# flavie-yuan-liu/DL_attack_on_ImageNet

Hardware: AMD Instinct MI355X
Metric: adversarial images/sec (ADiL learning step, classifier included) (higher is better)
Workload: dtype bf16; 1 GPU; ADiL learn_dictionary_a step vs resnet50, 512 images/GPU, 50 atoms, 224x224, bf16 image streams + fp32 D/V master, loss=logits, clean pseudo-labels computed once per image and cached (1 fwd + 1 bwd per step; result-neutral, profiles/r03_label_stability.md); global_batch=512, atoms=50, inner_iters=132, parallelism=dp1: images+codes sharded, D replicated, 1 all-reduce(grad_d)/step

## Files before the change

dl_attack_on_imagenet_amd/csrc/adil_stem.hip:

```cpp
#include <hip/hip_runtime.h>
#include <stdint.h>

#include "adil_common.h"
#include "adil_hip.h"
#include "adil_mfma.h"

namespace {

struct StemNorm { float mean[3]; float inv_std[3]; };

#define ST_T 16
#define ST_ROWS (2 * ST_T + 5)
#define ST_COLS 40
#define ST_RS (ST_COLS * 4 + 8)
#define ST_K 224
#define ST_WS (ST_K + 8)
#define ST_OS 72

template <typename TX>
__global__ __launch_bounds__(256) __attribute__((amdgpu_waves_per_eu(3))) void stem_conv_fwd_kernel(const TX* __restrict__ x, const bf16_t* __restrict__ wf,
                                                            StemNorm nm, const float* __restrict__ scale,
                                                            const float* __restrict__ shift, bf16_t* __restrict__ y,
                                                            int H, int W, int OH, int OW) {
    __shared__ __attribute__((aligned(16))) bf16_t smem[ST_ROWS * ST_RS + 64 * ST_WS];
    static_assert(4 * 32 * ST_OS <= ST_ROWS * ST_RS + 64 * ST_WS, "output scratch must fit in the tile buffers");
    bf16_t* sin = smem;
    bf16_t* sw = smem + ST_ROWS * ST_RS;
    bf16_t* sout = smem;
    const int tid = threadIdx.x, lane = tid & 63, w = tid >> 6, c = lane & 31, h = lane >> 5;
    const int n = blockIdx.z, oh0 = blockIdx.y * ST_T, ow0 = blockIdx.x * ST_T;
    {
        u32x4 wv[7];
#pragma unroll
        for (int j = 0; j < 7; ++j) wv[j] = *reinterpret_cast<const u32x4*>(wf + (size_t)(tid + 256 * j) * 8);
#pragma unroll
        for (int j = 0; j < 7; ++j) {
            const int q = tid + 256 * j, co = q / 28, off = q - co * 28;
            *reinterpret_cast<u32x4*>(sw + co * ST_WS + off * 8) = wv[j];
        }
    }
    const TX* xn = x + (size_t)n * 3 * H * W;
    constexpr int NPOS = (ST_ROWS * ST_COLS + 255) / 256;
    float raw[NPOS][3], okm[NPOS];
#pragma unroll
    for (int j = 0; j < NPOS; ++j) {
        const int pos = tid + 256 * j < ST_ROWS * ST_COLS ? tid + 256 * j : ST_ROWS * ST_COLS - 1;
        const int row = pos / ST_COLS, col = pos - row * ST_COLS;
        const int ih = 2 * oh0 - 3 + row, iw = 2 * ow0 - 3 + col;
        const bool ok = (ih >= 0) && (ih < H) && (iw >= 0) && (iw < W);
        const size_t at = (size_t)(ok ? ih : 0) * W + (ok ? iw : 0);
        okm[j] = ok ? 1.0f : 0.0f;
        raw[j][0] = Elem<TX>::load(xn, at);
        raw[j][1] = Elem<TX>::load(xn + (size_t)H * W, at);
        raw[j][2] = Elem<TX>::load(xn + (size_t)2 * H * W, at);
    }
#pragma unroll
    for (int j = 0; j < NPOS; ++j) {
        const int pos = tid + 256 * j;
        const int row = pos / ST_COLS, col = pos - row * ST_COLS;
        const float v0 = (raw[j][0] - nm.mean[0]) * nm.inv_std[0] * okm[j];
        const float v1 = (raw[j][1] - nm.mean[1]) * nm.inv_std[1] * okm[j];
        const float v2 = (raw[j][2] - nm.mean[2]) * nm.inv_std[2] * okm[j];
        u32x2 t;
        t[0] = pack2_bf16(v0, v1);
        t[1] = pack2_bf16(v2, 0.0f);
        if (pos < ST_ROWS * ST_COLS) *reinterpret_cast<u32x2*>(sin + row * ST_RS + col * 4) = t;
    }
    lds_sync();
    f32x16 acc[2][2];
#pragma unroll
    for (int p = 0; p < 2; ++p)
#pragma unroll
        for (int ct = 0; ct < 2; ++ct)
#pragma unroll
            for (int r = 0; r < 16; ++r) acc[p][ct][r] = 0.0f;
    const int prow = c >> 4, pcol = c & 15;
#pragma unroll 1
    for (int kh = 0; kh < 7; ++kh) {
#pragma unroll
        for (int g = 0; g < 2; ++g) {
            bf16x8 a[2], b[2];
#pragma unroll
            for (int ct = 0; ct < 2; ++ct) a[ct] = lds8(sw + (ct * 32 + c) * ST_WS + kh * 32 + 16 * g + 8 * h);
#pragma unroll
            for (int p = 0; p < 2; ++p) {
                const int orow = 2 * (2 * w + p) + prow;
                b[p] = lds8(sin + (2 * orow + kh) * ST_RS + 8 * pcol + 16 * g + 8 * h);
            }
#pragma unroll
            for (int p = 0; p < 2; ++p)
#pragma unroll
                for (int ct = 0; ct < 2; ++ct) mma16(acc[p][ct], a[ct], b[p]);
        }
    }
    lds_sync();
    bf16_t* so = sout + w * 32 * ST_OS;
#pragma unroll
    for (int p = 0; p < 2; ++p) {
#pragma unroll
        for (int ct = 0; ct < 2; ++ct) {
#pragma unroll
            for (int q = 0; q < 4; ++q) {
                const int co = ct * 32 + 8 * q + 4 * h;
                float v[4];
#pragma unroll
                for (int j = 0; j < 4; ++j) v[j] = fmaxf(acc[p][ct][4 * q + j] * scale[co + j] + shift[co + j], 0.0f);
                u32x2 t;
                t[0] = pack2_bf16(v[0], v[1]);
                t[1] = pack2_bf16(v[2], v[3]);
                *reinterpret_cast<u32x2*>(so + c * ST_OS + co) = t;
            }
        }
#pragma unroll
        for (int i = 0; i < 4; ++i) {
            const int id = lane + 64 * i, px = id >> 3, ch = (id & 7) * 8;
            const int oh = oh0 + 2 * (2 * w + p) + (px >> 4), ow = ow0 + (px & 15);
            const u32x4 t = *reinterpret_cast<const u32x4*>(so + px * ST_OS + ch);
            if (oh < OH && ow < OW) *reinterpret_cast<u32x4*>(y + (((size_t)n * OH + oh) * OW + ow) * 64 + ch) = t;
        }
    }
}


__global__ __launch_bounds__(256) void maxpool_fwd_kernel(const bf16_t* __restrict__ y, bf16_t* __restrict__ p,
                                                          uint8_t* __restrict__ idx, int B, int OH, int OW, int PH, int PW,
                                                          int C8) {
    const size_t i = (size_t)blockIdx.x * 256 + threadIdx.x;
    const size_t total = (size_t)B * PH * PW * C8;
    if (i >= total) return;
    const int c8 = (int)(i % C8);
    size_t r = i / C8;
    const int pw = (int)(r % PW); r /= PW;
    const int ph = (int)(r % PH);
    const int n = (int)(r / PH);
    float best[8];
    unsigned bi[8];
#pragma unroll
    for (int j = 0; j < 8; ++j) { best[j] = -INFINITY; bi[j] = 0xffu; }
#pragma unroll
    for (int kh = 0; kh < 3; ++kh) {
        const int oh = 2 * ph - 1 + kh;
#pragma unroll
        for (int kw = 0; kw < 3; ++kw) {
            const int ow = 2 * pw - 1 + kw;
            if (oh >= 0 && oh < OH && ow >= 0 && ow < OW) {
                const u32x4 t = *reinterpret_cast<const u32x4*>(y + ((((size_t)n * OH + oh) * OW + ow) * C8 + c8) * 8);
                float f[8];
                unpack8(t, f);
#pragma unroll
                for (int j = 0; j < 8; ++j) {
                    const bool take = (f[j] > best[j]) || (f[j] != f[j]) || (bi[j] == 0xffu);
                    best[j] = take ? f[j] : best[j];
                    bi[j] = take ? (unsigned)(kh * 3 + kw) : bi[j];
                }
            }
        }
    }
    *reinterpret_cast<u32x4*>(p + i * 8) = pack8(best);
    u32x2 o;
    o[0] = bi[0] | (bi[1] << 8) | (bi[2] << 16) | (bi[3] << 24);
    o[1] = bi[4] | (bi[5] << 8) | (bi[6] << 16) | (bi[7] << 24);
    *reinterpret_cast<u32x2*>(idx + i * 8) = o;
}

__global__ __launch_bounds__(256) void stem_pool_bwd_kernel(const bf16_t* __restrict__ g, const uint8_t* __restrict__ idx,
                                                            const bf16_t* __restrict__ p, const float* __restrict__ scale,
                                                            bf16_t* __restrict__ gy, int B, int OH, int OW, int PH, int PW,
                                                            int C8) {
    const size_t i = (size_t)blockIdx.x * 256 + threadIdx.x;
    const size_t total = (size_t)B * OH * OW * C8;
    if (i >= total) return;
    const int c8 = (int)(i % C8);
    size_t r = i / C8;
    const int ow = (int)(r % OW); r /= OW;
    const int oh = (int)(r % OH);
    const int n = (int)(r / OH);
    float acc[8];
#pragma unroll
    for (int j = 0; j < 8; ++j) acc[j] = 0.0f;
    const int ph0 = oh >> 1, nph = 1 + (oh & 1), pw0 = ow >> 1, npw = 1 + (ow & 1);
    for (int a = 0; a < nph; ++a) {
        const int ph = ph0 + a;
        if (ph >= PH) continue;
        const int kh = oh - (2 * ph - 1);
        for (int b = 0; b < npw; ++b) {
            const int pw = pw0 + b;
            if (pw >= PW) continue;
            const unsigned want = (unsigned)(kh * 3 + (ow - (2 * pw - 1)));
            const size_t at = ((((size_t)n * PH + ph) * PW + pw) * C8 + c8) * 8;
            const u32x2 id = *reinterpret_cast<const u32x2*>(idx + at);
            const u32x4 gt = *reinterpret_cast<const u32x4*>(g + at);
            const u32x4 pt = *reinterpret_cast<const u32x4*>(p + at);
            float gf[8], pf[8];
            unpack8(gt, gf);
            unpack8(pt, pf);
#pragma unroll
            for (int j = 0; j < 8; ++j) {
                const unsigned k = (id[j >> 2] >> (8 * (j & 3))) & 0xffu;
                acc[j] += (k == want && pf[j] > 0.0f) ? gf[j] : 0.0f;
            }
        }
    }
#pragma unroll
    for (int j = 0; j < 8; ++j) acc[j] *= scale[c8 * 8 + j];
    *reinterpret_cast<u32x4*>(gy + i * 8) = pack8(acc);
}

#define SB_TH 16
#define SB_TW 32
#define SB_GR (SB_TH / 2 + 3)
#define SB_GC (SB_TW / 2 + 3)
#define SB_PS 72

typedef float f32x4 __attribute__((ext_vector_type(4)));

template <int A, int BB>
__device__ __forceinline__ void stem_bwd_class(f32x4 (&acc)[2], const bf16_t* sg, const bf16_t* swb, int w, int l16, int ks) {
    const int wrow = (l16 < 3 ? l16 : 0) * 49 * 64;
    const bool wlane = l16 < 3;
#pragma unroll 1
    for (int kh = 1 - A; kh < 7; kh += 2) {
#pragma unroll
        for (int kw = 1 - BB; kw < 7; kw += 2) {
            const int col = l16 + (BB + 3 - kw) / 2 + 1;
#pragma unroll
            for (int cg = 0; cg < 2; ++cg) {
                bf16x8 a = {};
                if (wlane) a = lds8(swb + wrow + (kh * 7 + kw) * 64 + 32 * cg + 8 * ks);
#pragma unroll
                for (int q = 0; q < 2; ++q) {
                    const int row = 2 * w + q + (A + 3 - kh) / 2 + 1;
                    const bf16x8 b = lds8(sg + (row * SB_GC + col) * SB_PS + 32 * cg + 8 * ks);
                    acc[q] = __builtin_amdgcn_mfma_f32_16x16x32_bf16(a, b, acc[q], 0, 0, 0);
                }
            }
        }
    }
}

template <typename TX> __device__ __forceinline__ void st_pair(TX* p, float a, float b);
template <> __device__ __forceinline__ void st_pair<float>(float* p, float a, float b) {
    *reinterpret_cast<float2*>(p) = make_float2(a, b);
}
template <> __device__ __forceinline__ void st_pair<bf16_t>(bf16_t* p, float a, float b) {
    *reinterpret_cast<unsigned*>(p) = pack2_bf16(a, b);
}

template <typename TX>
__global__ __launch_bounds__(256) __attribute__((amdgpu_waves_per_eu(3))) void stem_conv_bwd_kernel(const bf16_t* __restrict__ gy, const bf16_t* __restrict__ wb,
                                                            StemNorm nm, TX* __restrict__ gx, int H, int W, int OH,
                                                            int OW) {
    __shared__ __attribute__((aligned(16))) bf16_t sg[SB_GR * SB_GC * SB_PS];
    __shared__ __attribute__((aligned(16))) bf16_t swb[3 * 49 * 64];
    const int tid = threadIdx.x, lane = tid & 63, w = tid >> 6, c = lane & 31, h = lane >> 5;
    const int n = blockIdx.z, ih0 = blockIdx.y * SB_TH, iw0 = blockIdx.x * SB_TW;
    {
        constexpr int NWQ = (3 * 49 * 8 + 255) / 256, NGQ = (SB_GR * SB_GC * 8 + 255) / 256;
        u32x4 wv[NWQ], gv[NGQ];
        bool gok[NGQ];
#pragma unroll
        for (int j = 0; j < NWQ; ++j) {
            const int q = tid + 256 * j < 3 * 49 * 8 ? tid + 256 * j : 3 * 49 * 8 - 1;
            wv[j] = *reinterpret_cast<const u32x4*>(wb + q * 8);
        }
        const int ohb = ih0 / 2 - 1, owb = iw0 / 2 - 1;
#pragma unroll
        for (int j = 0; j < NGQ; ++j) {
            const int q = tid + 256 * j < SB_GR * SB_GC * 8 ? tid + 256 * j : SB_GR * SB_GC * 8 - 1;
            const int ch = q & 7, px = q >> 3;
            const int row = px / SB_GC, col = px - row * SB_GC;
            const int oh = ohb + row, ow = owb + col;
            gok[j] = (oh >= 0) && (oh < OH) && (ow >= 0) && (ow < OW);
            gv[j] = *reinterpret_cast<const u32x4*>(gy + (((size_t)n * OH + (gok[j] ? oh : 0)) * OW + (gok[j] ? ow : 0)) * 64 + ch * 8);
        }
#pragma unroll
        for (int j = 0; j < NWQ; ++j) {
            const int q = tid + 256 * j;
            if (q < 3 * 49 * 8) *reinterpret_cast<u32x4*>(swb + q * 8) = wv[j];
        }
#pragma unroll
        for (int j = 0; j < NGQ; ++j) {
            const int q = tid + 256 * j;
            const int ch = q & 7, px = q >> 3;
            u32x4 t = gv[j];
            if (!gok[j]) t = u32x4{0u, 0u, 0u, 0u};
            if (q < SB_GR * SB_GC * 8) *reinterpret_cast<u32x4*>(sg + px * SB_PS + ch * 8) = t;
        }
    }
    lds_sync();
    const int l16 = lane & 15, ks = lane >> 4;
    f32x4 acc[4][2];
#pragma unroll
    for (int k = 0; k < 4; ++k)
#pragma unroll
        for (int q = 0; q < 2; ++q) acc[k][q] = f32x4{0.0f, 0.0f, 0.0f, 0.0f};
    stem_bwd_class<0, 0>(acc[0], sg, swb, w, l16, ks);
    stem_bwd_class<0, 1>(acc[1], sg, swb, w, l16, ks);
    stem_bwd_class<1, 0>(acc[2], sg, swb, w, l16, ks);
    stem_bwd_class<1, 1>(acc[3], sg, swb, w, l16, ks);
    if (ks == 0) {
        const int iw = iw0 + 2 * l16;
#pragma unroll
        for (int q = 0; q < 2; ++q) {
#pragma unroll
            for (int a = 0; a < 2; ++a) {
                const int ih = ih0 + 2 * (2 * w + q) + a;
                if (ih < H && iw < W) {
#pragma unroll
                    for (int ci = 0; ci < 3; ++ci) {
                        TX* o = gx + (((size_t)n * 3 + ci) * H + ih) * W + iw;
                        st_pair<TX>(o, acc[2 * a][q][ci] * nm.inv_std[ci], acc[2 * a + 1][q][ci] * nm.inv_std[ci]);
                    }
                }
            }
        }
    }
}

}

extern "C" int adil_stem_conv_fwd(const void* x, int x_dtype, const void* w_fwd, float mean0, float mean1, float mean2,
                                  float inv_std0, float inv_std1, float inv_std2, const float* scale, const float* shift,
                                  void* y, int B, int H, int W, void* stream) {
    ADIL_ENTER();
    if (!x || !w_fwd || !scale || !shift || !y || B <= 0 || H <= 0 || W <= 0 || (H & 1) || (W & 1)) return ADIL_EINVAL;
    const StemNorm nm = {{mean0, mean1, mean2}, {inv_std0, inv_std1, inv_std2}};
    const int OH = H / 2, OW = W / 2;
    const dim3 grid((OW + ST_T - 1) / ST_T, (OH + ST_T - 1) / ST_T, B);
    hipStream_t st = (hipStream_t)stream;
    if (x_dtype == ADIL_F32)
        hipLaunchKernelGGL(stem_conv_fwd_kernel<float>, grid, dim3(256), 0, st, (const float*)x, (const bf16_t*)w_fwd, nm,
                           scale, shift, (bf16_t*)y, H, W, OH, OW);
    else if (x_dtype == ADIL_BF16)
        hipLaunchKernelGGL(stem_conv_fwd_kernel<bf16_t>, grid, dim3(256), 0, st, (const bf16_t*)x, (const bf16_t*)w_fwd, nm,
                           scale, shift, (bf16_t*)y, H, W, OH, OW);
    else
        return ADIL_EINVAL;
    ADIL_CHECK_LAUNCH();
    return 0;
}

extern "C" int adil_maxpool_fwd(const void* y, void* p, uint8_t* idx, int B, int OH, int OW, int C, void* stream) {
    ADIL_ENTER();
    if (!y || !p || !idx || B <= 0 || OH <= 0 || OW <= 0 || C <= 0 || (C & 7)) return ADIL_EINVAL;
    const int PH = (OH - 1) / 2 + 1, PW = (OW - 1) / 2 + 1;
    const size_t total = (size_t)B * PH * PW * (C / 8);
    hipLaunchKernelGGL(maxpool_fwd_kernel, dim3((unsigned)((total + 255) / 256)), dim3(256), 0, (hipStream_t)stream,
                       (const bf16_t*)y, (bf16_t*)p, idx, B, OH, OW, PH, PW, C / 8);
    ADIL_CHECK_LAUNCH();
    return 0;
}

extern "C" int adil_stem_pool_bwd(const void* g, const uint8_t* idx, const void* p, const float* scale, void* gy, int B,
                                  int OH, int OW, int C, void* stream) {
    ADIL_ENTER();
    if (!g || !idx || !p || !scale || !gy || B <= 0 || OH <= 0 || OW <= 0 || C <= 0 || (C & 7)) return ADIL_EINVAL;
    const int PH = (OH - 1) / 2 + 1, PW = (OW - 1) / 2 + 1;
    const size_t total = (size_t)B * OH * OW * (C / 8);
    hipLaunchKernelGGL(stem_pool_bwd_kernel, dim3((unsigned)((total + 255) / 256)), dim3(256), 0, (hipStream_t)stream,
                       (const bf16_t*)g, idx, (const bf16_t*)p, scale, (bf16_t*)gy, B, OH, OW, PH, PW, C / 8);
    ADIL_CHECK_LAUNCH();
    return 0;
}

extern "C" int adil_stem_conv_bwd(const void* gy, const void* w_bwd, float inv_std0, float inv_std1, float inv_std2, void* gx,
                                  int gx_dtype, int B, int H, int W, void* stream) {
    ADIL_ENTER();
    if (!gy || !w_bwd || !gx || B <= 0 || H <= 0 || W <= 0 || (H & 1) || (W & 1)) return ADIL_EINVAL;
    const StemNorm nm = {{0.0f, 0.0f, 0.0f}, {inv_std0, inv_std1, inv_std2}};
    const int OH = H / 2, OW = W / 2;
    const dim3 grid((W + SB_TW - 1) / SB_TW, (H + SB_TH - 1) / SB_TH, B);
    hipStream_t st = (hipStream_t)stream;
    if (gx_dtype == ADIL_F32)
        hipLaunchKernelGGL(stem_conv_bwd_kernel<float>, grid, dim3(256), 0, st, (const bf16_t*)gy, (const bf16_t*)w_bwd, nm,
                           (float*)gx, H, W, OH, OW);
    else if (gx_dtype == ADIL_BF16)
        hipLaunchKernelGGL(stem_conv_bwd_kernel<bf16_t>, grid, dim3(256), 0, st, (const bf16_t*)gy, (const bf16_t*)w_bwd, nm,
                           (bf16_t*)gx, H, W, OH, OW);
    else
        return ADIL_EINVAL;
    ADIL_CHECK_LAUNCH();
    return 0;
}
```

Before: 22790 images/sec.

## Restructure stem conv backward loop with double-buffered LDS fragments and shared gradient loads

Rewrites the stem conv backward MFMA loop so that every gradient tile position loaded from LDS is shared across all four parity classes. The loop is fully unrolled, and the next iteration's A and B fragments are double-buffered in registers ahead of the MFMAs, with sched barriers enforcing the overlap. Each weight channel row in LDS is padded to reduce bank conflicts. The max-pool backward kernel now issues all four candidate loads at once, branch-free, and reads scale with vector loads. The cost is higher register pressure, which could lower occupancy under waves_per_eu(3).

```diff
diff --git a/dl_attack_on_imagenet_amd/csrc/adil_stem.hip b/dl_attack_on_imagenet_amd/csrc/adil_stem.hip
--- a/dl_attack_on_imagenet_amd/csrc/adil_stem.hip
+++ b/dl_attack_on_imagenet_amd/csrc/adil_stem.hip
@@ -175,34 +175,41 @@
     const int ow = (int)(r % OW); r /= OW;
     const int oh = (int)(r % OH);
     const int n = (int)(r / OH);
+    const int ph0 = oh >> 1, pw0 = ow >> 1;
+    u32x2 id[4];
+    u32x4 gt[4], pt[4];
+    bool ok[4];
+#pragma unroll
+    for (int q = 0; q < 4; ++q) {
+        const int a = q >> 1, b = q & 1;
+        ok[q] = (a <= (oh & 1)) && (b <= (ow & 1)) && (ph0 + a < PH) && (pw0 + b < PW);
+        const int ph = ok[q] ? ph0 + a : ph0, pw = ok[q] ? pw0 + b : pw0;
+        const size_t at = ((((size_t)n * PH + ph) * PW + pw) * C8 + c8) * 8;
+        id[q] = *reinterpret_cast<const u32x2*>(idx + at);
+        gt[q] = *reinterpret_cast<const u32x4*>(g + at);
+        pt[q] = *reinterpret_cast<const u32x4*>(p + at);
+    }
+    const float4 s0 = *reinterpret_cast<const float4*>(scale + c8 * 8);
+    const float4 s1 = *reinterpret_cast<const float4*>(scale + c8 * 8 + 4);
+    const float sc[8] = {s0.x, s0.y, s0.z, s0.w, s1.x, s1.y, s1.z, s1.w};
     float acc[8];
 #pragma unroll
     for (int j = 0; j < 8; ++j) acc[j] = 0.0f;
-    const int ph0 = oh >> 1, nph = 1 + (oh & 1), pw0 = ow >> 1, npw = 1 + (ow & 1);
-    for (int a = 0; a < nph; ++a) {
-        const int ph = ph0 + a;
-        if (ph >= PH) continue;
-        const int kh = oh - (2 * ph - 1);
-        for (int b = 0; b < npw; ++b) {
-            const int pw = pw0 + b;
-            if (pw >= PW) continue;
-            const unsigned want = (unsigned)(kh * 3 + (ow - (2 * pw - 1)));
-            const size_t at = ((((size_t)n * PH + ph) * PW + pw) * C8 + c8) * 8;
-            const u32x2 id = *reinterpret_cast<const u32x2*>(idx + at);
-            const u32x4 gt = *reinterpret_cast<const u32x4*>(g + at);
-            const u32x4 pt = *reinterpret_cast<const u32x4*>(p + at);
-            float gf[8], pf[8];
-            unpack8(gt, gf);
-            unpack8(pt, pf);
-#pragma unroll
-            for (int j = 0; j < 8; ++j) {
-                const unsigned k = (id[j >> 2] >> (8 * (j & 3))) & 0xffu;
-                acc[j] += (k == want && pf[j] > 0.0f) ? gf[j] : 0.0f;
-            }
-        }
-    }
-#pragma unroll
-    for (int j = 0; j < 8; ++j) acc[j] *= scale[c8 * 8 + j];
+#pragma unroll
+    for (int q = 0; q < 4; ++q) {
+        const int a = q >> 1, b = q & 1;
+        const unsigned want = (unsigned)((oh - (2 * (ph0 + a) - 1)) * 3 + (ow - (2 * (pw0 + b) - 1)));
+        float gf[8], pf[8];
+        unpack8(gt[q], gf);
+        unpack8(pt[q], pf);
+#pragma unroll
+        for (int j = 0; j < 8; ++j) {
+            const unsigned k = (id[q][j >> 2] >> (8 * (j & 3))) & 0xffu;
+            acc[j] += (ok[q] & (k == want) & (pf[j] > 0.0f)) ? gf[j] : 0.0f;
+        }
+    }
+#pragma unroll
+    for (int j = 0; j < 8; ++j) acc[j] *= sc[j];
     *reinterpret_cast<u32x4*>(gy + i * 8) = pack8(acc);
 }
 
@@ -211,32 +218,9 @@
 #define SB_GR (SB_TH / 2 + 3)
 #define SB_GC (SB_TW / 2 + 3)
 #define SB_PS 72
+#define SB_WC (49 * 64 + 16)
 
 typedef float f32x4 __attribute__((ext_vector_type(4)));
-
-template <int A, int BB>
-__device__ __forceinline__ void stem_bwd_class(f32x4 (&acc)[2], const bf16_t* sg, const bf16_t* swb, int w, int l16, int ks) {
-    const int wrow = (l16 < 3 ? l16 : 0) * 49 * 64;
-    const bool wlane = l16 < 3;
-#pragma unroll 1
-    for (int kh = 1 - A; kh < 7; kh += 2) {
-#pragma unroll
-        for (int kw = 1 - BB; kw < 7; kw += 2) {
-            const int col = l16 + (BB + 3 - kw) / 2 + 1;
-#pragma unroll
-            for (int cg = 0; cg < 2; ++cg) {
-                bf16x8 a = {};
-                if (wlane) a = lds8(swb + wrow + (kh * 7 + kw) * 64 + 32 * cg + 8 * ks);
-#pragma unroll
-                for (int q = 0; q < 2; ++q) {
-                    const int row = 2 * w + q + (A + 3 - kh) / 2 + 1;
-                    const bf16x8 b = lds8(sg + (row * SB_GC + col) * SB_PS + 32 * cg + 8 * ks);
-                    acc[q] = __builtin_amdgcn_mfma_f32_16x16x32_bf16(a, b, acc[q], 0, 0, 0);
-                }
-            }
-        }
-    }
-}
 
 template <typename TX> __device__ __forceinline__ void st_pair(TX* p, float a, float b);
 template <> __device__ __forceinline__ void st_pair<float>(float* p, float a, float b) {
@@ -251,8 +235,8 @@
                                                             StemNorm nm, TX* __restrict__ gx, int H, int W, int OH,
                                                             int OW) {
     __shared__ __attribute__((aligned(16))) bf16_t sg[SB_GR * SB_GC * SB_PS];
-    __shared__ __attribute__((aligned(16))) bf16_t swb[3 * 49 * 64];
-    const int tid = threadIdx.x, lane = tid & 63, w = tid >> 6, c = lane & 31, h = lane >> 5;
+    __shared__ __attribute__((aligned(16))) bf16_t swb[3 * SB_WC];
+    const int tid = threadIdx.x, lane = tid & 63, w = tid >> 6;
     const int n = blockIdx.z, ih0 = blockIdx.y * SB_TH, iw0 = blockIdx.x * SB_TW;
     {
         constexpr int NWQ = (3 * 49 * 8 + 255) / 256, NGQ = (SB_GR * SB_GC * 8 + 255) / 256;
@@ -275,8 +259,8 @@
         }
 #pragma unroll
         for (int j = 0; j < NWQ; ++j) {
-            const int q = tid + 256 * j;
-            if (q < 3 * 49 * 8) *reinterpret_cast<u32x4*>(swb + q * 8) = wv[j];
+            const int q = tid + 256 * j, ci = q / (49 * 8);
+            if (q < 3 * 49 * 8) *reinterpret_cast<u32x4*>(swb + ci * SB_WC + (q - ci * 49 * 8) * 8) = wv[j];
         }
 #pragma unroll
         for (int j = 0; j < NGQ; ++j) {
@@ -289,15 +273,47 @@
     }
     lds_sync();
     const int l16 = lane & 15, ks = lane >> 4;
-    f32x4 acc[4][2];
-#pragma unroll
-    for (int k = 0; k < 4; ++k)
-#pragma unroll
-        for (int q = 0; q < 2; ++q) acc[k][q] = f32x4{0.0f, 0.0f, 0.0f, 0.0f};
-    stem_bwd_class<0, 0>(acc[0], sg, swb, w, l16, ks);
-    stem_bwd_class<0, 1>(acc[1], sg, swb, w, l16, ks);
-    stem_bwd_class<1, 0>(acc[2], sg, swb, w, l16, ks);
-    stem_bwd_class<1, 1>(acc[3], sg, swb, w, l16, ks);
+    const bf16_t* ap = swb + (l16 < 3 ? l16 : 0) * SB_WC + 8 * ks;
+    const bf16_t* bp = sg + (2 * w * SB_GC + l16) * SB_PS + 8 * ks;
+    f32x4 acc[2][2][2];
+#pragma unroll
+    for (int k = 0; k < 8; ++k) (&acc[0][0][0])[k] = f32x4{0.0f, 0.0f, 0.0f, 0.0f};
+    bf16x8 bfr[2][2][2], afr[2][2][2][2];
+#pragma unroll
+    for (int i = -1; i < 16; ++i) {
+        if (i + 1 < 16) {
+            const int off = 3 - (i + 1) / 4, s = 3 - (i + 1) % 4, nb = (i + 1) & 1;
+#pragma unroll
+            for (int q = 0; q < 2; ++q)
+#pragma unroll
+                for (int cg = 0; cg < 2; ++cg) bfr[nb][q][cg] = lds8(bp + ((q + off) * SB_GC + s) * SB_PS + 32 * cg);
+#pragma unroll
+            for (int a = 0; a < 2; ++a)
+#pragma unroll
+                for (int bb = 0; bb < 2; ++bb) {
+                    const int t = bb + 2 - s, kh = a + 5 - 2 * off, kw = 1 - bb + 2 * t;
+                    if (off > 2 + a || t < 0) continue;
+#pragma unroll
+                    for (int cg = 0; cg < 2; ++cg) afr[nb][a][bb][cg] = lds8(ap + (kh * 7 + kw) * 64 + 32 * cg);
+                }
+        }
+        __builtin_amdgcn_sched_barrier(0);
+        if (i >= 0) {
+            const int off = 3 - i / 4, s = 3 - i % 4, cb = i & 1;
+#pragma unroll
+            for (int cg = 0; cg < 2; ++cg)
+#pragma unroll
+                for (int a = 0; a < 2; ++a)
+#pragma unroll
+                    for (int bb = 0; bb < 2; ++bb) {
+                        if (off > 2 + a || bb + 2 - s < 0) continue;
+#pragma unroll
+                        for (int q = 0; q < 2; ++q)
+                            acc[a][bb][q] = __builtin_amdgcn_mfma_f32_16x16x32_bf16(afr[cb][a][bb][cg], bfr[cb][q][cg], acc[a][bb][q], 0, 0, 0);
+                    }
+        }
+        __builtin_amdgcn_sched_barrier(0);
+    }
     if (ks == 0) {
         const int iw = iw0 + 2 * l16;
 #pragma unroll
@@ -309,7 +325,7 @@
 #pragma unroll
                     for (int ci = 0; ci < 3; ++ci) {
                         TX* o = gx + (((size_t)n * 3 + ci) * H + ih) * W + iw;
-                        st_pair<TX>(o, acc[2 * a][q][ci] * nm.inv_std[ci], acc[2 * a + 1][q][ci] * nm.inv_std[ci]);
+                        st_pair<TX>(o, acc[a][0][q][ci] * nm.inv_std[ci], acc[a][1][q][ci] * nm.inv_std[ci]);
                     }
                 }
             }
```

After: 23270 images/sec (median of 6 runs). +2.1%, better.
